# marqo-ai/marqo

Hardware: AMD Instinct MI355X
Metric: embeddings/sec (higher is better)
Workload: dtype bf16; 1 GPU; open_clip ViT-B/32 image tower, uint8 224x224 resident in HBM (tower-only), batch 256/GPU; global_batch=256, parallelism=dp1 (replicated weights, sharded items, RCCL all_gather of embeddings), weights=random-init (seed 0) ViT-B-32, last_block_rows=pooled

## Files before the change

marqo_amd/csrc/attn_proj.hip:

```cpp
#include "common.h"
#include "gemm_loop.h"

typedef short s16x4 __attribute__((ext_vector_type(4)));
typedef unsigned u32x2 __attribute__((ext_vector_type(2)));

extern mq_knob mq_xcd_band;
extern mq_knob mq_ln_prefetch;
int mq_device_ok();

namespace {

template <int OFF>
__device__ __forceinline__ s16x4 lds_read_tr16(unsigned addr) {
    s16x4 v;
    asm volatile("ds_read_b64_tr_b16 %0, %1 offset:%2" : "=v"(v) : "v"(addr), "n"(OFF));
    return v;
}
template <int OFF>
__device__ __forceinline__ bf16x8 gload16(const void* p) {
    i32x4 v;
    asm volatile("global_load_dwordx4 %0, %1, off offset:%2" : "=v"(v) : "v"(p), "n"(OFF));
    return __builtin_bit_cast(bf16x8, v);
}
struct ApPrefetch { const unsigned* a; const unsigned* b; unsigned na, nb; };
__device__ __forceinline__ void lds_write8(unsigned addr, u32x2 v) { asm volatile("ds_write_b64 %0, %1" ::"v"(addr), "v"(v) : "memory"); }

__device__ __forceinline__ float fold_sum(float v) {
    const auto r = __builtin_amdgcn_permlane16_swap(__float_as_uint(v), __float_as_uint(v), false, false);
    const float w = __uint_as_float(r[0]) + __uint_as_float(r[1]);
    const auto q = __builtin_amdgcn_permlane32_swap(__float_as_uint(w), __float_as_uint(w), false, false);
    return __uint_as_float(q[0]) + __uint_as_float(q[1]);
}
__device__ __forceinline__ float fold_max(float v) {
    const auto r = __builtin_amdgcn_permlane16_swap(__float_as_uint(v), __float_as_uint(v), false, false);
    const float w = fmaxf(__uint_as_float(r[0]), __uint_as_float(r[1]));
    const auto q = __builtin_amdgcn_permlane32_swap(__float_as_uint(w), __float_as_uint(w), false, false);
    return fmaxf(__uint_as_float(q[0]), __uint_as_float(q[1]));
}

constexpr int AP_TILE = 8192;
constexpr int AP_KV = 32768;
constexpr int AP_RING = 65536;

template <int W>
__global__ __launch_bounds__(512, 1) void attn_proj_kernel(const bf16_t* __restrict__ qkv, const bf16_t* __restrict__ Wo, const float* __restrict__ bias,
                                                            bf16_t* x, float2* __restrict__ rowstats, int len, float scale_log2e, float inv_w, float eps, int band, ApPrefetch pf, int dbg) {
    static_assert(W % 256 == 0 && (W / 64) % 2 == 0, "whole 256-column thirds, heads in pairs");
    constexpr int NHEAD = W / 64, NG = NHEAD / 2, NT3 = W / 256;
    constexpr int PANEL = NHEAD * AP_TILE;
    extern __shared__ __attribute__((aligned(16))) char smem[];
    const int tid = threadIdx.x, lane = tid & 63;
    const int wave = __builtin_amdgcn_readfirstlane(tid >> 6);
    const int l15 = lane & 15, g = lane >> 4;
    const unsigned img = xcd_banded_block(blockIdx.x, gridDim.x, band);
    const int64_t row0 = (int64_t)img * len;
    constexpr int ld = 3 * W;
    const bf16_t* qkv0 = qkv + row0 * ld;
    const unsigned lds0 = (unsigned)(uintptr_t)(__attribute__((address_space(3))) char*)smem;
    const unsigned ring = lds0 + PANEL;

    const int hl = wave >> 2, qblk = wave & 3;
    const bool active = qblk * 16 < len;
    auto stage = [&](int grp) {
        char* buf = smem + PANEL + (grp & 1) * AP_KV;
#pragma unroll
        for (int i = 0; i < 4; ++i) {
            const int p = wave * 4 + i;
            const int ph = p >> 4, is_v = (p >> 3) & 1, piece = p & 7;
            const int row = piece * 8 + (lane >> 3);
            const int key = row < len ? row : len - 1;
            const int lc = (lane & 7) ^ (row & 7);
            const bf16_t* src = qkv0 + (int64_t)key * ld + (is_v ? 2 * W : W) + (2 * grp + ph) * 64 + lc * 8;
            __builtin_amdgcn_global_load_lds((const __attribute__((address_space(1))) void*)src,
                                             (__attribute__((address_space(3))) void*)(buf + ph * 16384 + is_v * 8192 + piece * 1024), 16, 0, 0);
        }
    };
    const int qi = qblk * 16 + l15;
    const int64_t q_off = (int64_t)(qi < len ? qi : len - 1) * ld + hl * 64 + 8 * g;
    auto load_q = [&](int grp, bf16x8 (&q)[2]) {
        const bf16_t* qb = qkv0 + q_off + grp * 128;
        q[0] = gload16<0>(qb);
        q[1] = gload16<64>(qb);
    };
    const unsigned k_sw0 = (unsigned)(l15 * 128 + ((g ^ (l15 & 7)) << 4)), k_sw1 = (unsigned)(l15 * 128 + (((g + 4) ^ (l15 & 7)) << 4));
    const int vkey = 4 * g + (l15 >> 2), vcol = (l15 & 3) >> 1, vhalf = (l15 & 1) << 3;
    unsigned v_off[4];
#pragma unroll
    for (int dt = 0; dt < 4; ++dt) v_off[dt] = (unsigned)(8192 + vkey * 128 + ((((dt << 1) | vcol) ^ (vkey & 7)) << 4) + vhalf);
    unsigned o_off[4];
#pragma unroll
    for (int dt = 0; dt < 4; ++dt) o_off[dt] = (unsigned)(qi * 128 + (((dt * 2 + (g >> 1)) ^ (qi & 7)) << 4) + (g & 1) * 8);

    i32x4 res[4][NT3];
#pragma unroll
    for (int mt = 0; mt < 4; ++mt)
#pragma unroll
        for (int a = 0; a < NT3; ++a) res[mt][a] = i32x4{0, 0, 0, 0};
    unsigned pf_reg[2] = {0u, 0u};
    const unsigned pf_nt = gridDim.x * 512u, pf_t = blockIdx.x * 512u + (unsigned)tid;

    bf16x8 qn[2] = {bf16x8{0, 0, 0, 0, 0, 0, 0, 0}, bf16x8{0, 0, 0, 0, 0, 0, 0, 0}};
    if (!(dbg & 1)) {
    stage(0);
    load_q(0, qn);
    asm volatile("s_waitcnt vmcnt(0)" ::: "memory");
    landed(qn[0]); landed(qn[1]);
    static_for<NG>([&](auto grp_tag) {
        constexpr int grp = decltype(grp_tag)::value;
        __builtin_amdgcn_s_barrier();
        asm volatile("" ::: "memory");
        bf16x8 qf[2] = {qn[0], qn[1]};
        if constexpr (grp + 1 < NG) {
            stage(grp + 1);
            load_q(grp + 1, qn);
        }
        if constexpr (grp < 4) {
            const int m = grp * 16 + l15;
            const bf16_t* xr = x + (row0 + (m < len ? m : 0)) * W + wave * (W / 8) + (g & 1) * 16 + (g >> 1) * 8;
            static_for<NT3>([&](auto a_tag) {
                constexpr int a = decltype(a_tag)::value;
                res[grp][a] = __builtin_bit_cast(i32x4, gload16<a * 64>(xr));
            });
        }
        if constexpr (grp == 1 || grp == 3) {
            constexpr int j = grp >> 1;
// ... 89 lines not shown
    asm volatile("s_waitcnt lgkmcnt(0)" ::: "memory");
    __builtin_amdgcn_s_barrier();
    asm volatile("" ::: "memory");

    const unsigned slot0 = ring + (unsigned)wave * 8192u;
    const unsigned w_rd0 = (unsigned)(l15 * 128 + ((g ^ (l15 & 7)) << 4)), w_rd1 = (unsigned)(l15 * 128 + (((g + 4) ^ (l15 & 7)) << 4));
    const unsigned w_vo = (unsigned)((lane >> 3) * (W * 2) + (((lane & 7) ^ ((lane >> 3) & 7)) << 4));
    constexpr unsigned W_BYTES = (unsigned)W * W * 2;
    auto issue_unit = [&](int kt, int i, int slot, bool live) {
        const unsigned rec = live ? W_BYTES : 0u;
        const unsigned soff = (unsigned)((wave * (W / 8) + i * 16) * (W * 2) + kt * 128);
        const auto rs = __builtin_amdgcn_make_buffer_rsrc((void*)Wo, 0, rec, 0x00020000);
        dma16(rs, w_vo, soff, slot0 + (unsigned)slot * 2048u);
        dma16(rs, w_vo + 8u * (W * 2), soff, slot0 + (unsigned)slot * 2048u + 1024u);
    };
    f32x4 acc[NT3][4][2];
#pragma unroll
    for (int a = 0; a < NT3; ++a)
#pragma unroll
        for (int mt = 0; mt < 4; ++mt) { acc[a][mt][0] = f32x4{0.f, 0.f, 0.f, 0.f}; acc[a][mt][1] = f32x4{0.f, 0.f, 0.f, 0.f}; }
    constexpr int UPK = 2 * NT3;
    constexpr int UPI = 2 * UPK;
    static_assert(UPI % 4 == 0, "slot indices must be static inside an iteration");
    bf16x8 tf[4][2], wf[2][2];
    issue_unit(0, 0, 0, true);
    issue_unit(0, 1, 1, true);
    issue_unit(0, 2, 2, true);
    issue_unit(0, 3, 3, true);
    static_for<4>([&](auto mt_tag) {
        constexpr int mt = decltype(mt_tag)::value;
        tf[mt][0] = lds_read16<mt * 2048>(lds0 + w_rd0);
        tf[mt][1] = lds_read16<mt * 2048>(lds0 + w_rd1);
    });
    asm volatile("s_waitcnt vmcnt(6)" ::: "memory");
    wf[0][0] = lds_read16<0>(slot0 + w_rd0);
    wf[0][1] = lds_read16<0>(slot0 + w_rd1);
    for (int ktp = 0; ktp < ((dbg & 2) ? 0 : NHEAD / 2); ++ktp) {
        static_for<UPI>([&](auto ii_tag) {
            constexpr int ii = decltype(ii_tag)::value, i = ii % UPK, cur = ii & 1, slot = ii & 3;
            const int kt = 2 * ktp + ii / UPK;
            asm volatile("s_waitcnt lgkmcnt(0)" ::: "memory");
            landed(wf[cur][0]); landed(wf[cur][1]);
            if constexpr (i == 0) {
#pragma unroll
                for (int mt = 0; mt < 4; ++mt) { landed(tf[mt][0]); landed(tf[mt][1]); }
            }
            __builtin_amdgcn_sched_barrier(0);
            constexpr int a = i >> 1, j = i & 1;
#pragma unroll
            for (int mt = 0; mt < 4; ++mt) {
                acc[a][mt][j] = __builtin_amdgcn_mfma_f32_16x16x32_bf16(wf[cur][0], tf[mt][0], acc[a][mt][j], 0, 0, 0);
                acc[a][mt][j] = __builtin_amdgcn_mfma_f32_16x16x32_bf16(wf[cur][1], tf[mt][1], acc[a][mt][j], 0, 0, 0);
            }
            __builtin_amdgcn_sched_barrier(0);
            {
                constexpr int i4 = (ii + 4) % UPI;
                const int ktp4 = ktp + (ii + 4) / UPI;
                issue_unit(2 * ktp4 + i4 / UPK, i4 % UPK, slot, ktp4 < NHEAD / 2);
            }
            asm volatile("s_waitcnt vmcnt(6)" ::: "memory");
            {
                constexpr int nslot = (ii + 1) & 3;
                wf[cur ^ 1][0] = lds_read16<nslot * 2048>(slot0 + w_rd0);
                wf[cur ^ 1][1] = lds_read16<nslot * 2048>(slot0 + w_rd1);
            }
            if constexpr (i == UPK - 1) {
                __builtin_amdgcn_sched_barrier(0);
                const unsigned tb = lds0 + (unsigned)(kt + 1 < NHEAD ? kt + 1 : kt) * AP_TILE;
                static_for<4>([&](auto mt_tag) {
                    constexpr int mt = decltype(mt_tag)::value;
                    tf[mt][0] = lds_read16<mt * 2048>(tb + w_rd0);
                    tf[mt][1] = lds_read16<mt * 2048>(tb + w_rd1);
                });
            }
        });
    }
    asm volatile("s_waitcnt vmcnt(0)" ::: "memory");
    asm volatile("s_waitcnt lgkmcnt(0)" ::: "memory");
    landed(wf[0][0]); landed(wf[0][1]); landed(wf[1][0]); landed(wf[1][1]);
#pragma unroll
    for (int mt = 0; mt < 4; ++mt) { landed(tf[mt][0]); landed(tf[mt][1]); }

    if (dbg & 4) return;
    constexpr int WC = W / 8;
    f32x4 bias_v[NT3][2];
#pragma unroll
    for (int a = 0; a < NT3; ++a)
#pragma unroll
        for (int j = 0; j < 2; ++j) bias_v[a][j] = *(const f32x4*)(bias + wave * WC + a * 32 + j * 16 + 4 * g);
    char* mine = smem + PANEL + wave * 8192;
    const bool odd = (wave & 1) != 0;
    auto chain_add = [](f32x2_t& s1, f32x2_t& s2, unsigned px, unsigned py) {
        const f32x2_t e0 = {__uint_as_float(px << 16), __uint_as_float(px & 0xffff0000u)}, e1 = {__uint_as_float(py << 16), __uint_as_float(py & 0xffff0000u)};
        s1 += e0 + e1;
        s2 = __builtin_elementwise_fma(e0, e0, __builtin_elementwise_fma(e1, e1, s2));
    };
    unsigned held[4][4];
#pragma unroll
    for (int mt = 0; mt < 4; ++mt) {
        const int m = mt * 16 + l15;
        const bool m_ok = m < len;
        bf16_t* xr = x + (row0 + (m_ok ? m : 0)) * W + wave * WC;
        f32x2_t w1 = {0.f, 0.f}, w2 = {0.f, 0.f};
        f32x2_t h1 = {0.f, 0.f}, h2 = {0.f, 0.f};
#pragma unroll
        for (int a = 0; a < NT3; ++a) {
            uint2 pk[2];
            const auto q0 = __builtin_amdgcn_permlane16_swap((unsigned)res[mt][a][0], (unsigned)res[mt][a][2], false, false);
            const auto q1 = __builtin_amdgcn_permlane16_swap((unsigned)res[mt][a][1], (unsigned)res[mt][a][3], false, false);
#pragma unroll
            for (int j = 0; j < 2; ++j) {
                f32x4 v = acc[a][mt][j];
                v += bias_v[a][j];
                const unsigned rq[2] = {q0[j], q1[j]};
                v += f32x4{__uint_as_float(rq[0] << 16), __uint_as_float(rq[0] & 0xffff0000u), __uint_as_float(rq[1] << 16), __uint_as_float(rq[1] & 0xffff0000u)};
                pk[j].x = pack_bf16x2(v[0], v[1]);
                pk[j].y = pack_bf16x2(v[2], v[3]);
                const unsigned px = m_ok ? pk[j].x : 0u, py = m_ok ? pk[j].y : 0u;
                if constexpr (NT3 == 3) {
                    if (a == 1) chain_add(w1, w2, px, py);
                    else if (a == 0) {
                        if (odd) { held[mt][2 * j] = px; held[mt][2 * j + 1] = py; }
                        else chain_add(w1, w2, px, py);
                    } else {
                        if (odd) chain_add(w1, w2, px, py);
                        else chain_add(h1, h2, px, py);
                    }
                }
            }
            const auto r0 = __builtin_amdgcn_permlane16_swap(pk[0].x, pk[1].x, false, false);
            const auto r1 = __builtin_amdgcn_permlane16_swap(pk[0].y, pk[1].y, false, false);
            if (m_ok) *(uint4*)(xr + a * 32 + (g & 1) * 16 + (g >> 1) * 8) = make_uint4(r0[0], r1[0], r0[1], r1[1]);
        }
        if (rowstats) {
            const float st1 = fold_sum(w1[0] + w1[1]), st2 = fold_sum(w2[0] + w2[1]);
            if (g == 0) ((float2*)mine)[m] = make_float2(st1, st2);
            if (!odd) ((f32x4*)(mine + 1024))[mt * 64 + lane] = f32x4{h1[0], h1[1], h2[0], h2[1]};
        }
    }
    if (rowstats) {
        static_assert(NT3 == 3, "the slot hand-over is written for 96 columns per wave");
        __syncthreads();
        if (odd) {
            const f32x4* theirs = (const f32x4*)(smem + PANEL + (wave - 1) * 8192 + 1024);
#pragma unroll
            for (int mt = 0; mt < 4; ++mt) {
                const f32x4 st = theirs[mt * 64 + lane];
                f32x2_t h1 = {st[0], st[1]}, h2 = {st[2], st[3]};
                chain_add(h1, h2, held[mt][0], held[mt][1]);
                chain_add(h1, h2, held[mt][2], held[mt][3]);
                const float st1 = fold_sum(h1[0] + h1[1]), st2 = fold_sum(h2[0] + h2[1]);
                if (g == 0) ((float2*)(mine + 512))[mt * 16 + l15] = make_float2(st1, st2);
            }
        }
        __syncthreads();
        if (tid < len) {
            float s1 = 0.f, s2 = 0.f;
#pragma unroll
            for (int slot = 0; slot < W / 64; ++slot) {
                const int k = slot / 3, r = slot % 3;
                const char* src = smem + PANEL + (2 * k + (r ? 1 : 0)) * 8192 + (r == 1 ? 512 : 0);
                const float2 p = ((const float2*)src)[tid];
                s1 += p.x;
                s2 += p.y;
            }
            rowstats[row0 + tid] = mq_finalize_stats(s1, s2, inv_w, eps);
        }
    }
}

}

extern "C" int mq_attention_proj_ok(int64_t nseq, int32_t fixed_len, int32_t W, int32_t heads) {
    return nseq >= 1 && fixed_len >= 1 && fixed_len <= 64 && W == 768 && heads == 12 && nseq * fixed_len < (1LL << 31);
}

extern "C" int mq_attention_proj(const void* d_qkv, const void* d_w, const float* d_bias, void* d_x, float* d_rowstats, int64_t nseq, int32_t fixed_len, int32_t W,
                                 int32_t heads, float eps, const void* d_pf_a, size_t pf_a_bytes, const void* d_pf_b, size_t pf_b_bytes, void* stream) {
    MQ_CHECK_ARG(d_qkv && d_w && d_bias && d_x, "mq_attention_proj: null operand");
    MQ_CHECK_ARG(mq_attention_proj_ok(nseq, fixed_len, W, heads), "mq_attention_proj: takes 1..64-token sequences of a 768-wide tower with 12 heads (nseq=%ld len=%d W=%d heads=%d)",
                 (long)nseq, fixed_len, W, heads);
    MQ_CHECK_ARG((((uintptr_t)d_qkv | (uintptr_t)d_w | (uintptr_t)d_x | (uintptr_t)d_bias) & 15) == 0, "mq_attention_proj: operands must be 16-byte aligned");
    MQ_TRY(mq_device_ok());
    hipStream_t s = (hipStream_t)stream;
    constexpr int LDS = 12 * AP_TILE + AP_RING;
    static std::atomic<uint64_t> attr_done{0};
    auto kern = attn_proj_kernel<768>;
    if (hipError_t e = mq_ensure_dyn_lds((const void*)kern, LDS, attr_done); e != hipSuccess) {
        mq_set_error("mq_attention_proj: hipFuncSetAttribute: %s", hipGetErrorString(e));
        return MQ_ERR_HIP;
    }
    ApPrefetch pf{nullptr, nullptr, 0u, 0u};
    if (mq_ln_prefetch && nseq * fixed_len >= 1024) {
        auto lines = [](const void* p, size_t b) { return (p && ((uintptr_t)p & 3) == 0 && b < ((size_t)1 << 30)) ? (unsigned)(b / 128) : 0u; };
        pf.a = (const unsigned*)d_pf_a; pf.na = lines(d_pf_a, pf_a_bytes);
        pf.b = (const unsigned*)d_pf_b; pf.nb = lines(d_pf_b, pf_b_bytes);
    }
    static const bool dbg_on = getenv("MQ_AP_DEBUG") != nullptr;
    const char* dbg_s = dbg_on ? getenv("MQ_AP_DEBUG") : nullptr;
    const int dbg = dbg_s ? atoi(dbg_s) : 0;
    MqProfScope prof(2, s);
    const float scale_log2e = 1.44269504088896340736f / sqrtf(64.0f);
    hipLaunchKernelGGL(kern, dim3((unsigned)nseq), dim3(512), LDS, s, (const bf16_t*)d_qkv, (const bf16_t*)d_w, d_bias, (bf16_t*)d_x, (float2*)d_rowstats, (int)fixed_len,
                       scale_log2e, 1.0f / (float)W, eps, (mq_xcd_band && nseq >= 256) ? 1 : 0, pf, dbg);
    MQ_CHECK_LAUNCH("mq_attention_proj");
    return MQ_OK;
}
```

marqo_amd/csrc/gemm_bf16.hip:

```cpp
#include <map>
#include <mutex>
#include <string>
#include <type_traits>
#include "common.h"
#include "gemm_epilogue.h"
#include "gemm_loop.h"
#include "gemm_sched.h"

extern mq_knob mq_tower_row_select;
extern mq_knob mq_tower_ln_fold;
extern mq_knob mq_tower_subln_fold;
extern mq_knob mq_tower_attn_proj;
extern mq_knob mq_tower_panel_gemm;
extern mq_knob mq_attention_waves;
extern mq_knob mq_tower_residual_bf16;
extern mq_knob mq_gemm_small_max_rows;
bool mq_gemm_small_ok(int64_t M, int64_t N, int64_t K, bool ln);
bool mq_gemm_small_grouped_ok(int64_t M, int64_t N, int64_t K);
extern mq_knob mq_gemm_small_group_rows;
extern mq_knob mq_ln_prefetch;
int mq_gemm_small(const void* d_A, int64_t lda, const void* d_W, int64_t ldw, const float* d_bias, const void* d_residual, void* d_out,
                  int64_t ldc, int64_t M, int64_t N, int64_t K, int flags, hipStream_t s);
int mq_gemm_wd_launch(int flags, int mt, int ns, const void* A, int64_t lda, const void* W, int64_t ldw, const float* bias, const float* residual, void* out,
                      int64_t ldc, int M, int N, int K, const GemmGeom& g, int wide, const GemmLn& ln, hipStream_t s);

int mq_device_ok();

namespace {

struct GemmSk {
    float* partials;
    unsigned* flags;
    unsigned epoch;
    int tail_splits;
};

template <int FLAGS, int MT, int NH, int WM, int ORD>
__global__ __launch_bounds__(128 * WM, (NH == 1 && WM == 2) ? 2 : 1) void gemm_nt_kernel(
    const bf16_t* __restrict__ A, int64_t lda, const bf16_t* __restrict__ Wt, int64_t ldw,
    const float* __restrict__ bias, const float* residual, void* out, int64_t ldc,
    int M, int N, int K, int tiles_n, int num_tiles, int cgroup, int band_rows, int wide_store,
    unsigned a_bytes, unsigned w_bytes, GemmLn ln, GemmSk sk) {
    static_assert(!(NH == 2 && WM == 2), "the 4-wave 224 x 256 tile (one wave per SIMD) lost on every shape (profiles/r05a, r05b) and was removed in round 6");
    constexpr int BM = 16 * MT * WM, BN = 128 * NH;
    constexpr bool TAIL = WM == 4;
    constexpr int NTW = 4 * NH;
    constexpr int A_TILE_BYTES = BM * BK * 2, W_TILE_BYTES = BN * BK * 2;
    constexpr int STAGE_BYTES = A_TILE_BYTES + W_TILE_BYTES;
    constexpr int NPA = MT, NPW = 8 * NH / WM;
    constexpr int NLD = NPA + NPW;
    constexpr int NLR = MT + NTW;
    constexpr int NM = NTW * MT;
    constexpr bool LN_RES = (FLAGS & MQ_EPI_LN_APPLY) && (FLAGS & MQ_EPI_RESIDUAL);
    constexpr int ERG = !(FLAGS & MQ_EPI_RESIDUAL) ? MT : LN_RES ? ((NH == 2 || WM == 4) ? 1 : MT <= 4 ? MT : 2) : (NH == 2 || WM == 4) ? MT
                        : (FLAGS & MQ_EPI_OUT_F32) ? (MT <= 3 ? MT : (MT + 1) / 2) : (MT <= 5 ? MT : 3);
    extern __shared__ __attribute__((aligned(16))) char smem[];

    const GemmTileMap<BM, BN> tile_map(num_tiles, tiles_n, M, cgroup, band_rows);

    const int tid = threadIdx.x;
    const int lane = tid & 63;
    const int wave = __builtin_amdgcn_readfirstlane(tid >> 6);
    const int wm = wave >> 1, wn = wave & 1;
    const int l15 = lane & 15, g = lane >> 4;

    const int srow = lane >> 3;
    const unsigned chunk_off = (unsigned)(((lane & 7) ^ (srow & 7)) * 16);
    unsigned a_vo[NPA], w_vo[NPW];
    auto set_sources = [&](int m0, int n0) {
#pragma unroll
        for (int i = 0; i < MT; ++i) {
            int gm = m0 + wave * (8 * MT) + i * 8 + srow; gm = gm < M ? gm : M - 1;
            a_vo[i] = (unsigned)gm * (unsigned)lda * 2u + chunk_off;
        }
#pragma unroll
        for (int i = 0; i < NPW; ++i) {
            int gn = n0 + wave * (8 * NPW) + i * 8 + srow; gn = gn < N ? gn : N - 1;
            w_vo[i] = (unsigned)gn * (unsigned)ldw * 2u + chunk_off;
        }
    };
    const int nk = K / BK;
    int d_vbid = blockIdx.x, d_k = 0;
    unsigned a_rec = a_bytes, w_rec = w_bytes;
    bool tail_mode = false;
    int d_left = 0;
    const bool has_main = !TAIL || (int)blockIdx.x < num_tiles;
    if (has_main) {
        int m0, n0;
        tile_map.origin(d_vbid, m0, n0);
        set_sources(m0, n0);
    } else {
        a_rec = 0; w_rec = 0;
#pragma unroll
        for (int i = 0; i < NPA; ++i) a_vo[i] = 0;
#pragma unroll
        for (int i = 0; i < NPW; ++i) w_vo[i] = 0;
    }
    const unsigned lds0 = (unsigned)(uintptr_t)(__attribute__((address_space(3))) char*)smem;
    const unsigned dma_a0 = lds0 + (unsigned)wave * (8 * MT * 128), dma_w0 = lds0 + A_TILE_BYTES + (unsigned)wave * (8 * NPW * 128);
    auto issue_piece = [&](int i, unsigned bufoff) {
        const unsigned soff = (unsigned)d_k * (BK * 2);
        if (i < NPA) dma16(__builtin_amdgcn_make_buffer_rsrc((void*)A, 0, a_rec, 0x00020000), a_vo[i < NPA ? i : 0], soff, dma_a0 + bufoff + (unsigned)i * 1024u);
        else dma16(__builtin_amdgcn_make_buffer_rsrc((void*)Wt, 0, w_rec, 0x00020000), w_vo[i >= NPA ? i - NPA : 0], soff, dma_w0 + bufoff + (unsigned)(i - NPA) * 1024u);
// ... 493 lines not shown
    MqProfScope prof(0, s, 2.0 * (double)M * (double)N * (double)K);
    GemmLn ln{};
    ln.partials = (float2*)d_partials;
    ln.nslots = (int)((N + 63) / 64);
    ln.part_ld = M;
    return launch_gemm<MQ_EPI_BIAS | MQ_EPI_RESIDUAL | MQ_EPI_ROW_STATS>(d_A, lda, d_W, ldw, d_bias, (const float*)d_residual, d_out, ldc, (int)M, (int)N, (int)K, s, ln);
}

extern "C" int mq_gemm_bf16_lnrs(const void* d_A, int64_t lda, const void* d_W, int64_t ldw, const float* d_bias, const float* d_colsum, const float* d_rowstats,
                                 const void* d_residual, void* d_out, int64_t ldc, int64_t M, int64_t N, int64_t K, int flags, float* d_partials, void* stream) {
    MQ_CHECK_ARG(d_A && d_W && d_out && d_bias && d_colsum && d_rowstats && d_partials, "mq_gemm_bf16_lnrs: null operand");
    MQ_CHECK_ARG(flags == (MQ_EPI_BIAS | MQ_EPI_RESIDUAL) || flags == (MQ_EPI_BIAS | MQ_EPI_GLU), "mq_gemm_bf16_lnrs: flags must be MQ_EPI_BIAS | MQ_EPI_RESIDUAL or MQ_EPI_BIAS | MQ_EPI_GLU");
    MQ_CHECK_ARG(!(flags & MQ_EPI_RESIDUAL) || d_residual, "mq_gemm_bf16_lnrs: MQ_EPI_RESIDUAL without residual");
    MQ_TRY(check_shape("mq_gemm_bf16_lnrs", M, N, K, lda, ldw, ldc));
    MQ_CHECK_ARG(!(flags & MQ_EPI_GLU) || N % 32 == 0, "mq_gemm_bf16_lnrs: MQ_EPI_GLU needs N %% 32 == 0");
    hipStream_t s = (hipStream_t)stream;
    MqProfScope prof(0, s, 2.0 * (double)M * (double)N * (double)K);
    GemmLn ln{};
    ln.colsum = d_colsum;
    ln.rowstats = (const float2*)d_rowstats;
    ln.partials = (float2*)d_partials;
    ln.nslots = (int)((N + 63) / 64);
    ln.part_ld = M;
    if (flags & MQ_EPI_GLU)
        return launch_gemm<MQ_EPI_BIAS | MQ_EPI_GLU | MQ_EPI_LN_APPLY | MQ_EPI_ROW_STATS>(d_A, lda, d_W, ldw, d_bias, nullptr, d_out, ldc, (int)M, (int)N, (int)K, s, ln);
    return launch_gemm<MQ_EPI_BIAS | MQ_EPI_RESIDUAL | MQ_EPI_LN_APPLY | MQ_EPI_ROW_STATS>(d_A, lda, d_W, ldw, d_bias, (const float*)d_residual, d_out, ldc, (int)M, (int)N, (int)K, s, ln);
}

int mq_row_stats_finalize_pf(const float* d_partials, int32_t nslots, float* d_stats, int64_t rows, int32_t W, float eps, const void* pf_a, size_t bytes_a,
                             const void* pf_b, size_t bytes_b, hipStream_t s);
extern "C" int64_t mq_gemm_band_counters(int64_t M) { return M / 32 + 16; }
bool mq_gemm_rs_in_launch() { return g_tune.rs_fin && !g_tune.tail; }
extern "C" int mq_gemm_bf16_rsf(const void* d_A, int64_t lda, const void* d_W, int64_t ldw, const float* d_bias, const void* d_residual, void* d_out,
                                int64_t ldc, int64_t M, int64_t N, int64_t K, int flags, float* d_partials, float* d_stats, float eps,
                                uint32_t* d_band_ctr, const void* d_pf_a, size_t pf_a_bytes, const void* d_pf_b, size_t pf_b_bytes, void* stream) {
    MQ_CHECK_ARG(d_A && d_W && d_out && d_bias && d_residual && d_partials && d_stats, "mq_gemm_bf16_rsf: null operand");
    MQ_CHECK_ARG((flags | MQ_EPI_ROW_STATS) == (MQ_EPI_BIAS | MQ_EPI_RESIDUAL | MQ_EPI_ROW_STATS), "mq_gemm_bf16_rsf: flags must be MQ_EPI_BIAS | MQ_EPI_RESIDUAL");
    MQ_TRY(check_shape("mq_gemm_bf16_rsf", M, N, K, lda, ldw, ldc));
    hipStream_t s = (hipStream_t)stream;
    const int nslots = (int)((N + 63) / 64);
    const bool in_launch = d_band_ctr && g_tune.rs_fin && !g_tune.tail;
    {
        MqProfScope prof(0, s, 2.0 * (double)M * (double)N * (double)K);
        GemmLn ln{};
        ln.partials = (float2*)d_partials;
        ln.nslots = nslots;
        ln.part_ld = M;
        if (in_launch) {
            ln.band_ctr = d_band_ctr;
            ln.stats_out = (float2*)d_stats;
            ln.inv_w = 1.0f / (float)N;
            ln.eps = eps;
            ln.pf_a = (const unsigned*)d_pf_a;
            ln.pf_b = (const unsigned*)d_pf_b;
            ln.pf_na = d_pf_a ? (unsigned)(pf_a_bytes / 128) : 0u;
            ln.pf_nb = d_pf_b ? (unsigned)(pf_b_bytes / 128) : 0u;
        }
        MQ_TRY(launch_gemm<MQ_EPI_BIAS | MQ_EPI_RESIDUAL | MQ_EPI_ROW_STATS>(d_A, lda, d_W, ldw, d_bias, (const float*)d_residual, d_out, ldc, (int)M, (int)N, (int)K, s, ln));
    }
    if (in_launch) return MQ_OK;
    return mq_row_stats_finalize_pf(d_partials, nslots, d_stats, M, (int32_t)N, eps, d_pf_a, pf_a_bytes, d_pf_b, pf_b_bytes, s);
}

extern "C" int mq_tune(const char* key, int value) {
    MQ_CHECK_ARG(key, "mq_tune: null key");
    const std::string k(key);
    if (k == "gemm_mt") g_tune.mt = value;
    else if (k == "gemm_cgroup") g_tune.cgroup = value;
    else if (k == "gemm_nh") { g_tune.nh = value; g_tune.fp8_big = value == 4 ? 0 : value; }
    else if (k == "gemm_tail") g_tune.tail = value;
    else if (k == "gemm_wd") g_tune.wd = value;
    else if (k == "rs_finalize") g_tune.rs_fin = value;
    else if (k == "row_select") mq_tower_row_select = value;
    else if (k == "ln_fold") mq_tower_ln_fold = value;
    else if (k == "subln_fold") mq_tower_subln_fold = value;
    else if (k == "attn_proj") mq_tower_attn_proj = value;
    else if (k == "panel_gemm") mq_tower_panel_gemm = value;
    else if (k == "xcd_band") mq_xcd_band = value;
    else if (k == "attn_waves") mq_attention_waves = value;
    else if (k == "residual_bf16") mq_tower_residual_bf16 = value;
    else if (k == "small_m") mq_gemm_small_max_rows = value;
    else if (k == "small_m_grouped") mq_gemm_small_group_rows = value;
    else if (k == "ln_prefetch") mq_ln_prefetch = value;
    else if (k == "gemm_addr_limit_mb") mq_gemm_addr_limit = value > 0 ? ((uint64_t)value << 20) - 1 : 0xffffffffull;
    else { mq_set_error("mq_tune: unknown key %s", key); return MQ_ERR_INVALID; }
    return MQ_OK;
}
#endif
```

Before: 98150 embeddings/s.

## Interleave attention head-pairs with out-projection GEMM in fused attn_proj kernel

```diff
diff --git a/marqo_amd/csrc/attn_proj.hip b/marqo_amd/csrc/attn_proj.hip
--- a/marqo_amd/csrc/attn_proj.hip
+++ b/marqo_amd/csrc/attn_proj.hip
@@ -7,6 +7,7 @@
 extern mq_knob mq_xcd_band;
 extern mq_knob mq_ln_prefetch;
 int mq_device_ok();
+mq_knob mq_attn_proj_overlap{getenv("MQ_ATTN_PROJ_OVERLAP") ? atoi(getenv("MQ_ATTN_PROJ_OVERLAP")) : 1};
 
 namespace {
 
@@ -41,6 +42,97 @@
 constexpr int AP_TILE = 8192;
 constexpr int AP_KV = 32768;
 constexpr int AP_RING = 65536;
+
+template <int W>
+__device__ __forceinline__ void ap_epilogue(f32x4 (&acc)[W / 256][4][2], i32x4 (&res)[4][W / 256], const float* __restrict__ bias, bf16_t* x, float2* __restrict__ rowstats,
+                                            int64_t row0, int len, float inv_w, float eps, char* scratch, int tid, int lane, int wave, int l15, int g) {
+    constexpr int NT3 = W / 256;
+    constexpr int WC = W / 8;
+    f32x4 bias_v[NT3][2];
+#pragma unroll
+    for (int a = 0; a < NT3; ++a)
+#pragma unroll
+        for (int j = 0; j < 2; ++j) bias_v[a][j] = *(const f32x4*)(bias + wave * WC + a * 32 + j * 16 + 4 * g);
+    char* mine = scratch + wave * 8192;
+    const bool odd = (wave & 1) != 0;
+    auto chain_add = [](f32x2_t& s1, f32x2_t& s2, unsigned px, unsigned py) {
+        const f32x2_t e0 = {__uint_as_float(px << 16), __uint_as_float(px & 0xffff0000u)}, e1 = {__uint_as_float(py << 16), __uint_as_float(py & 0xffff0000u)};
+        s1 += e0 + e1;
+        s2 = __builtin_elementwise_fma(e0, e0, __builtin_elementwise_fma(e1, e1, s2));
+    };
+    unsigned held[4][4];
+#pragma unroll
+    for (int mt = 0; mt < 4; ++mt) {
+        const int m = mt * 16 + l15;
+        const bool m_ok = m < len;
+        bf16_t* xr = x + (row0 + (m_ok ? m : 0)) * W + wave * WC;
+        f32x2_t w1 = {0.f, 0.f}, w2 = {0.f, 0.f};
+        f32x2_t h1 = {0.f, 0.f}, h2 = {0.f, 0.f};
+#pragma unroll
+        for (int a = 0; a < NT3; ++a) {
+            uint2 pk[2];
+            const auto q0 = __builtin_amdgcn_permlane16_swap((unsigned)res[mt][a][0], (unsigned)res[mt][a][2], false, false);
+            const auto q1 = __builtin_amdgcn_permlane16_swap((unsigned)res[mt][a][1], (unsigned)res[mt][a][3], false, false);
+#pragma unroll
+            for (int j = 0; j < 2; ++j) {
+                f32x4 v = acc[a][mt][j];
+                v += bias_v[a][j];
+                const unsigned rq[2] = {q0[j], q1[j]};
+                v += f32x4{__uint_as_float(rq[0] << 16), __uint_as_float(rq[0] & 0xffff0000u), __uint_as_float(rq[1] << 16), __uint_as_float(rq[1] & 0xffff0000u)};
+                pk[j].x = pack_bf16x2(v[0], v[1]);
+                pk[j].y = pack_bf16x2(v[2], v[3]);
+                const unsigned px = m_ok ? pk[j].x : 0u, py = m_ok ? pk[j].y : 0u;
+                if constexpr (NT3 == 3) {
+                    if (a == 1) chain_add(w1, w2, px, py);
+                    else if (a == 0) {
+                        if (odd) { held[mt][2 * j] = px; held[mt][2 * j + 1] = py; }
+                        else chain_add(w1, w2, px, py);
+                    } else {
+                        if (odd) chain_add(w1, w2, px, py);
+                        else chain_add(h1, h2, px, py);
+                    }
+                }
+            }
+            const auto r0 = __builtin_amdgcn_permlane16_swap(pk[0].x, pk[1].x, false, false);
+            const auto r1 = __builtin_amdgcn_permlane16_swap(pk[0].y, pk[1].y, false, false);
+            if (m_ok) *(uint4*)(xr + a * 32 + (g & 1) * 16 + (g >> 1) * 8) = make_uint4(r0[0], r1[0], r0[1], r1[1]);
+        }
+        if (rowstats) {
+            const float st1 = fold_sum(w1[0] + w1[1]), st2 = fold_sum(w2[0] + w2[1]);
+            if (g == 0) ((float2*)mine)[m] = make_float2(st1, st2);
+            if (!odd) ((f32x4*)(mine + 1024))[mt * 64 + lane] = f32x4{h1[0], h1[1], h2[0], h2[1]};
+        }
+    }
+    if (rowstats) {
+        static_assert(NT3 == 3, "the slot hand-over is written for 96 columns per wave");
+        __syncthreads();
+        if (odd) {
+            const f32x4* theirs = (const f32x4*)(scratch + (wave - 1) * 8192 + 1024);
+#pragma unroll
+            for (int mt = 0; mt < 4; ++mt) {
+                const f32x4 st = theirs[mt * 64 + lane];
+                f32x2_t h1 = {st[0], st[1]}, h2 = {st[2], st[3]};
+                chain_add(h1, h2, held[mt][0], held[mt][1]);
+                chain_add(h1, h2, held[mt][2], held[mt][3]);
+                const float st1 = fold_sum(h1[0] + h1[1]), st2 = fold_sum(h2[0] + h2[1]);
+                if (g == 0) ((float2*)(mine + 512))[mt * 16 + l15] = make_float2(st1, st2);
+            }
+        }
+        __syncthreads();
+        if (tid < len) {
+            float s1 = 0.f, s2 = 0.f;
+#pragma unroll
+            for (int slot = 0; slot < W / 64; ++slot) {
+                const int k = slot / 3, r = slot % 3;
+                const char* src = scratch + (2 * k + (r ? 1 : 0)) * 8192 + (r == 1 ? 512 : 0);
+                const float2 p = ((const float2*)src)[tid];
+                s1 += p.x;
+                s2 += p.y;
+            }
+            rowstats[row0 + tid] = mq_finalize_stats(s1, s2, inv_w, eps);
+        }
+    }
+}
 
 template <int W>
 __global__ __launch_bounds__(512, 1) void attn_proj_kernel(const bf16_t* __restrict__ qkv, const bf16_t* __restrict__ Wo, const float* __restrict__ bias,
@@ -296,91 +388,293 @@
     for (int mt = 0; mt < 4; ++mt) { landed(tf[mt][0]); landed(tf[mt][1]); }
 
     if (dbg & 4) return;
-    constexpr int WC = W / 8;
-    f32x4 bias_v[NT3][2];
+    ap_epilogue<W>(acc, res, bias, x, rowstats, row0, len, inv_w, eps, smem + PANEL, tid, lane, wave, l15, g);
+}
+
+template <int W, int DBG>
+__global__ __launch_bounds__(512, 1) void attn_proj_overlap_kernel(const bf16_t* __restrict__ qkv, const bf16_t* __restrict__ Wo, const float* __restrict__ bias,
+                                                                    bf16_t* x, float2* __restrict__ rowstats, int len, float scale_log2e, float inv_w, float eps, int band, ApPrefetch pf) {
+    static_assert(W % 256 == 0 && (W / 64) % 2 == 0, "whole 256-column thirds, heads in pairs");
+    constexpr int NHEAD = W / 64, NG = NHEAD / 2, NT3 = W / 256;
+    constexpr int OBUF = 4 * AP_TILE;
+    constexpr int KVOFF = OBUF, RINGOFF = OBUF + 2 * AP_KV;
+    extern __shared__ __attribute__((aligned(16))) char smem[];
+    const int tid = threadIdx.x, lane = tid & 63;
+    const int wave = __builtin_amdgcn_readfirstlane(tid >> 6);
+    const int l15 = lane & 15, g = lane >> 4;
+    const unsigned img = xcd_banded_block(blockIdx.x, gridDim.x, band);
+    const int64_t row0 = (int64_t)img * len;
+    constexpr int ld = 3 * W;
+    const bf16_t* qkv0 = qkv + row0 * ld;
+    const unsigned lds0 = (unsigned)(uintptr_t)(__attribute__((address_space(3))) char*)smem;
+
+    const int hl = wave >> 2, qblk = wave & 3;
+    const bool active = qblk * 16 < len;
+    auto stage = [&](int grp, int half) {
+        char* buf = smem + KVOFF + (grp & 1) * AP_KV;
+#pragma unroll
+        for (int i = 2 * half; i < 2 * half + 2; ++i) {
+            const int p = wave * 4 + i;
+            const int ph = p >> 4, is_v = (p >> 3) & 1, piece = p & 7;
+            const int row = piece * 8 + (lane >> 3);
+            const int key = row < len ? row : len - 1;
+            const int lc = (lane & 7) ^ (row & 7);
+            const unsigned off = (unsigned)(key * ld + (is_v ? 2 * W : W) + ph * 64 + lc * 8) * 2u;
+            const char* src = (const char*)qkv0 + off + grp * 256;
+            __builtin_amdgcn_global_load_lds((const __attribute__((address_space(1))) void*)src,
+                                             (__attribute__((address_space(3))) void*)(buf + ph * 16384 + is_v * 8192 + piece * 1024), 16, 0, 0);
+        }
+    };
+    const int qi = qblk * 16 + l15;
+    const unsigned q_off = (unsigned)((qi < len ? qi : len - 1) * ld + hl * 64 + 8 * g) * 2u;
+    auto load_q = [&](int grp, bf16x8 (&q)[2]) {
+        const char* qb = (const char*)qkv0 + q_off + grp * 256;
+        q[0] = gload16<0>(qb);
+        q[1] = gload16<64>(qb);
+    };
+    const unsigned k_sw0 = (unsigned)(l15 * 128 + ((g ^ (l15 & 7)) << 4));
+    const int vkey = 4 * g + (l15 >> 2), vcol = (l15 & 3) >> 1, vhalf = (l15 & 1) << 3;
+    const unsigned v_off0 = (unsigned)(8192 + vkey * 128 + ((vcol ^ (vkey & 7)) << 4) + vhalf);
+    const unsigned o_off0 = (unsigned)(qi * 128 + (((g >> 1) ^ (qi & 7)) << 4) + (g & 1) * 8);
+
+    constexpr int RES0 = NG - 2;
+    i32x4 res[4][NT3];
+#pragma unroll
+    for (int mt = 0; mt < 4; ++mt)
+#pragma unroll
+        for (int a = 0; a < NT3; ++a) res[mt][a] = i32x4{0, 0, 0, 0};
+    unsigned pf_reg[2] = {0u, 0u};
+    const unsigned pf_nt = gridDim.x * 512u, pf_t = blockIdx.x * 512u + (unsigned)tid;
+
+    const unsigned slot0 = lds0 + RINGOFF + (unsigned)wave * 8192u;
+    const unsigned w_vo = (unsigned)((lane >> 3) * (W * 2) + (((lane & 7) ^ ((lane >> 3) & 7)) << 4));
+    constexpr unsigned W_BYTES = (unsigned)W * W * 2;
+    auto issue_unit = [&](int kt, int i, int slot, bool live) {
+        const unsigned rec = live ? W_BYTES : 0u;
+        const unsigned soff = (unsigned)((wave * (W / 8) + i * 16) * (W * 2) + kt * 128);
+        const auto rs = __builtin_amdgcn_make_buffer_rsrc((void*)Wo, 0, rec, 0x00020000);
+        dma16(rs, w_vo, soff, slot0 + (unsigned)slot * 2048u);
+        dma16(rs, w_vo + 8u * (W * 2), soff, slot0 + (unsigned)slot * 2048u + 1024u);
+    };
+    f32x4 acc[NT3][4][2];
 #pragma unroll
     for (int a = 0; a < NT3; ++a)
 #pragma unroll
-        for (int j = 0; j < 2; ++j) bias_v[a][j] = *(const f32x4*)(bias + wave * WC + a * 32 + j * 16 + 4 * g);
-    char* mine = smem + PANEL + wave * 8192;
-    const bool odd = (wave & 1) != 0;
-    auto chain_add = [](f32x2_t& s1, f32x2_t& s2, unsigned px, unsigned py) {
-        const f32x2_t e0 = {__uint_as_float(px << 16), __uint_as_float(px & 0xffff0000u)}, e1 = {__uint_as_float(py << 16), __uint_as_float(py & 0xffff0000u)};
-        s1 += e0 + e1;
-        s2 = __builtin_elementwise_fma(e0, e0, __builtin_elementwise_fma(e1, e1, s2));
-    };
-    unsigned held[4][4];
-#pragma unroll
-    for (int mt = 0; mt < 4; ++mt) {
-        const int m = mt * 16 + l15;
-        const bool m_ok = m < len;
-        bf16_t* xr = x + (row0 + (m_ok ? m : 0)) * W + wave * WC;
-        f32x2_t w1 = {0.f, 0.f}, w2 = {0.f, 0.f};
-        f32x2_t h1 = {0.f, 0.f}, h2 = {0.f, 0.f};
-#pragma unroll
-        for (int a = 0; a < NT3; ++a) {
-            uint2 pk[2];
-            const auto q0 = __builtin_amdgcn_permlane16_swap((unsigned)res[mt][a][0], (unsigned)res[mt][a][2], false, false);
-            const auto q1 = __builtin_amdgcn_permlane16_swap((unsigned)res[mt][a][1], (unsigned)res[mt][a][3], false, false);
-#pragma unroll
-            for (int j = 0; j < 2; ++j) {
-                f32x4 v = acc[a][mt][j];
-                v += bias_v[a][j];
-                const unsigned rq[2] = {q0[j], q1[j]};
-                v += f32x4{__uint_as_float(rq[0] << 16), __uint_as_float(rq[0] & 0xffff0000u), __uint_as_float(rq[1] << 16), __uint_as_float(rq[1] & 0xffff0000u)};
-                pk[j].x = pack_bf16x2(v[0], v[1]);
-                pk[j].y = pack_bf16x2(v[2], v[3]);
-                const unsigned px = m_ok ? pk[j].x : 0u, py = m_ok ? pk[j].y : 0u;
-                if constexpr (NT3 == 3) {
-                    if (a == 1) chain_add(w1, w2, px, py);
-                    else if (a == 0) {
-                        if (odd) { held[mt][2 * j] = px; held[mt][2 * j + 1] = py; }
-                        else chain_add(w1, w2, px, py);
-                    } else {
-                        if (odd) chain_add(w1, w2, px, py);
-                        else chain_add(h1, h2, px, py);
+        for (int mt = 0; mt < 4; ++mt) { acc[a][mt][0] = f32x4{0.f, 0.f, 0.f, 0.f}; acc[a][mt][1] = f32x4{0.f, 0.f, 0.f, 0.f}; }
+    constexpr int UPK = 2 * NT3;
+    constexpr int UPR = 2 * UPK;
+    static_assert(UPR % 4 == 0 && UPR > 4, "slot indices must be static inside a round");
+    constexpr bool LOADS = !(DBG & 1), ATTN = !(DBG & 1) && !(DBG & 8), UNITS = !(DBG & 2);
+
+    bf16x8 qn[2] = {bf16x8{0, 0, 0, 0, 0, 0, 0, 0}, bf16x8{0, 0, 0, 0, 0, 0, 0, 0}};
+    bf16x8 tf[4][2], wf[2][2];
+    if constexpr (LOADS) {
+        stage(0, 0);
+        stage(0, 1);
+        load_q(0, qn);
+    }
+    if constexpr (UNITS) {
+        issue_unit(0, 0, 0, true);
+        issue_unit(0, 1, 1, true);
+        issue_unit(0, 2, 2, true);
+        issue_unit(0, 3, 3, true);
+    }
+    asm volatile("s_waitcnt vmcnt(0)" ::: "memory");
+    landed(qn[0]); landed(qn[1]);
+    if constexpr (UNITS) {
+        wf[0][0] = lds_read16<0>(slot0 + k_sw0);
+        wf[0][1] = lds_read16<0>(slot0 + (k_sw0 ^ 64u));
+    }
+    static_for<NG + 1>([&](auto r_tag) {
+        constexpr int r = decltype(r_tag)::value;
+        if constexpr (r == 1) asm volatile("s_waitcnt lgkmcnt(0)" ::: "memory");
+        __builtin_amdgcn_s_barrier();
+        asm volatile("" ::: "memory");
+        constexpr int n_a = !LOADS ? 0 : (r + 1 < NG ? 2 : 0) + (r == NG ? 2 * NT3 : r >= RES0 ? NT3 : 0) + ((r == 1 || r == 3) ? 1 : 0);
+        constexpr int n_b = (LOADS && r + 1 < NG) ? 4 : 0;
+        auto issue_b = [&]() {
+            if constexpr (n_b != 0) {
+                stage(r + 1, 1);
+                load_q(r + 1, qn);
+            }
+        };
+        if constexpr (LOADS) {
+            if constexpr (r + 1 < NG) stage(r + 1, 0);
+            if constexpr (r >= RES0) {
+                static_for<(r == NG ? 2 : 1)>([&](auto t_tag) {
+                    constexpr int mt = r - RES0 + decltype(t_tag)::value;
+                    const int m = mt * 16 + l15;
+                    const char* xr = (const char*)(x + row0 * W) + (unsigned)((m < len ? m : 0) * W + wave * (W / 8) + (g & 1) * 16 + (g >> 1) * 8) * 2u;
+                    static_for<NT3>([&](auto a_tag) {
+                        constexpr int a = decltype(a_tag)::value;
+                        res[mt][a] = __builtin_bit_cast(i32x4, gload16<a * 64>(xr));
+                    });
+                });
+            }
+            if constexpr (r == 1 || r == 3) {
+                constexpr int j = r >> 1;
+                const unsigned c = pf_t + j * pf_nt;
+                const unsigned* src = c < pf.na ? pf.a + (size_t)c * 32 : (c - pf.na < pf.nb ? pf.b + (size_t)(c - pf.na) * 32 : (const unsigned*)qkv0);
+                asm volatile("global_load_dword %0, %1, off" : "=v"(pf_reg[j]) : "v"(src));
+            }
+        }
+        auto b_landed = [&]() { landed(qn[0]); landed(qn[1]); };
+        auto a_landed = [&]() {
+            if constexpr (LOADS && r >= RES0) {
+#pragma unroll
+                for (int a = 0; a < NT3; ++a) landed(res[r - RES0][a]);
+                if constexpr (r == NG) {
+#pragma unroll
+                    for (int a = 0; a < NT3; ++a) landed(res[r - RES0 + 1][a]);
+                }
+            }
+            if constexpr (LOADS && (r == 1 || r == 3)) landed(pf_reg[r >> 1]);
+        };
+        if constexpr (ATTN && r < NG) {
+            if (active) {
+                const unsigned kvb = lds0 + KVOFF + (unsigned)(r & 1) * AP_KV + (unsigned)hl * 16384u;
+                f32x4 sc[4];
+                static_for<2>([&](auto h_tag) {
+                    constexpr int h = decltype(h_tag)::value;
+                    bf16x8 kf[2][2];
+                    static_for<2>([&](auto t_tag) {
+                        constexpr int t = decltype(t_tag)::value;
+                        kf[t][0] = lds_read16<(2 * h + t) * 2048>(kvb + k_sw0);
+                        kf[t][1] = lds_read16<(2 * h + t) * 2048>(kvb + (k_sw0 ^ 64u));
+                    });
+                    asm volatile("s_waitcnt lgkmcnt(0)" ::: "memory");
+#pragma unroll
+                    for (int t = 0; t < 2; ++t) {
+                        landed(kf[t][0]); landed(kf[t][1]);
+                        sc[2 * h + t] = f32x4{0.f, 0.f, 0.f, 0.f};
+#pragma unroll
+                        for (int kk = 0; kk < 2; ++kk) sc[2 * h + t] = __builtin_amdgcn_mfma_f32_16x16x32_bf16(kf[t][kk], qn[kk], sc[2 * h + t], 0, 0, 0);
                     }
-                }
-            }
-            const auto r0 = __builtin_amdgcn_permlane16_swap(pk[0].x, pk[1].x, false, false);
-            const auto r1 = __builtin_amdgcn_permlane16_swap(pk[0].y, pk[1].y, false, false);
-            if (m_ok) *(uint4*)(xr + a * 32 + (g & 1) * 16 + (g >> 1) * 8) = make_uint4(r0[0], r1[0], r0[1], r1[1]);
-        }
-        if (rowstats) {
-            const float st1 = fold_sum(w1[0] + w1[1]), st2 = fold_sum(w2[0] + w2[1]);
-            if (g == 0) ((float2*)mine)[m] = make_float2(st1, st2);
-            if (!odd) ((f32x4*)(mine + 1024))[mt * 64 + lane] = f32x4{h1[0], h1[1], h2[0], h2[1]};
-        }
-    }
-    if (rowstats) {
-        static_assert(NT3 == 3, "the slot hand-over is written for 96 columns per wave");
-        __syncthreads();
-        if (odd) {
-            const f32x4* theirs = (const f32x4*)(smem + PANEL + (wave - 1) * 8192 + 1024);
-#pragma unroll
-            for (int mt = 0; mt < 4; ++mt) {
-                const f32x4 st = theirs[mt * 64 + lane];
-                f32x2_t h1 = {st[0], st[1]}, h2 = {st[2], st[3]};
-                chain_add(h1, h2, held[mt][0], held[mt][1]);
-                chain_add(h1, h2, held[mt][2], held[mt][3]);
-                const float st1 = fold_sum(h1[0] + h1[1]), st2 = fold_sum(h2[0] + h2[1]);
-                if (g == 0) ((float2*)(mine + 512))[mt * 16 + l15] = make_float2(st1, st2);
-            }
-        }
-        __syncthreads();
-        if (tid < len) {
-            float s1 = 0.f, s2 = 0.f;
-#pragma unroll
-            for (int slot = 0; slot < W / 64; ++slot) {
-                const int k = slot / 3, r = slot % 3;
-                const char* src = smem + PANEL + (2 * k + (r ? 1 : 0)) * 8192 + (r == 1 ? 512 : 0);
-                const float2 p = ((const float2*)src)[tid];
-                s1 += p.x;
-                s2 += p.y;
-            }
-            rowstats[row0 + tid] = mq_finalize_stats(s1, s2, inv_w, eps);
-        }
-    }
+                });
+                s16x4 vt[2][4];
+                auto read_v = [&](auto u_tag) {
+                    constexpr int u = decltype(u_tag)::value;
+                    static_for<4>([&](auto dt_tag) {
+                        constexpr int dt = decltype(dt_tag)::value;
+                        vt[0][dt] = lds_read_tr16<u * 4096>(kvb + (v_off0 ^ (unsigned)(dt << 5)));
+                        vt[1][dt] = lds_read_tr16<u * 4096 + 2048>(kvb + (v_off0 ^ (unsigned)(dt << 5)));
+                    });
+                };
+                read_v(std::integral_constant<int, 0>{});
+                if (len < 64) {
+#pragma unroll
+                    for (int t = 0; t < 4; ++t)
+#pragma unroll
+                        for (int q = 0; q < 4; ++q) sc[t][q] = (t * 16 + g * 4 + q < len) ? sc[t][q] : -INFINITY;
+                }
+                float mx = fmaxf(fmaxf(fmaxf(sc[0][0], sc[0][1]), fmaxf(sc[0][2], sc[0][3])), fmaxf(fmaxf(sc[1][0], sc[1][1]), fmaxf(sc[1][2], sc[1][3])));
+                mx = fmaxf(mx, fmaxf(fmaxf(fmaxf(sc[2][0], sc[2][1]), fmaxf(sc[2][2], sc[2][3])), fmaxf(fmaxf(sc[3][0], sc[3][1]), fmaxf(sc[3][2], sc[3][3]))));
+                mx = fold_max(mx);
+                const float neg_mc = -mx * scale_log2e;
+                float psum = 0.f;
+#pragma unroll
+                for (int t = 0; t < 4; ++t)
+#pragma unroll
+                    for (int q = 0; q < 4; ++q) {
+                        sc[t][q] = __builtin_amdgcn_exp2f(fmaf(sc[t][q], scale_log2e, neg_mc));
+                        psum += sc[t][q];
+                    }
+                f32x4 o[4];
+#pragma unroll
+                for (int dt = 0; dt < 4; ++dt) o[dt] = f32x4{0.f, 0.f, 0.f, 0.f};
+                static_for<2>([&](auto u_tag) {
+                    constexpr int u = decltype(u_tag)::value;
+                    asm volatile("s_waitcnt lgkmcnt(0)" ::: "memory");
+#pragma unroll
+                    for (int t = 0; t < 2; ++t)
+#pragma unroll
+                        for (int dt = 0; dt < 4; ++dt) landed(vt[t][dt]);
+                    union { uint32_t w[4]; bf16x8 v; } pb;
+                    pb.w[0] = pack_bf16x2(sc[2 * u][0], sc[2 * u][1]);
+                    pb.w[1] = pack_bf16x2(sc[2 * u][2], sc[2 * u][3]);
+                    pb.w[2] = pack_bf16x2(sc[2 * u + 1][0], sc[2 * u + 1][1]);
+                    pb.w[3] = pack_bf16x2(sc[2 * u + 1][2], sc[2 * u + 1][3]);
+#pragma unroll
+                    for (int dt = 0; dt < 4; ++dt) {
+                        union { s16x4 t[2]; bf16x8 v; } vf;
+                        vf.t[0] = vt[0][dt];
+                        vf.t[1] = vt[1][dt];
+                        o[dt] = __builtin_amdgcn_mfma_f32_16x16x32_bf16(vf.v, pb.v, o[dt], 0, 0, 0);
+                    }
+                    if constexpr (u == 0) {
+                        __builtin_amdgcn_sched_barrier(0);
+                        read_v(std::integral_constant<int, 1>{});
+                    }
+                });
+                const float inv = 1.0f / fold_sum(psum);
+                const unsigned ot = lds0 + (unsigned)(2 * (r & 1) + hl) * AP_TILE;
+#pragma unroll
+                for (int dt = 0; dt < 4; ++dt) {
+                    u32x2 p;
+                    p[0] = pack_bf16x2(o[dt][0] * inv, o[dt][1] * inv);
+                    p[1] = pack_bf16x2(o[dt][2] * inv, o[dt][3] * inv);
+                    lds_write8(ot + (o_off0 ^ (unsigned)(dt << 5)), p);
+                }
+            }
+        }
+        if constexpr (UNITS && r >= 1) {
+            constexpr unsigned ob = (unsigned)(2 * ((r - 1) & 1)) * AP_TILE;
+            static_for<4>([&](auto mt_tag) {
+                constexpr int mt = decltype(mt_tag)::value;
+                tf[mt][0] = lds_read16<mt * 2048>(lds0 + ob + k_sw0);
+                tf[mt][1] = lds_read16<mt * 2048>(lds0 + ob + (k_sw0 ^ 64u));
+            });
+            static_for<UPR>([&](auto ii_tag) {
+                constexpr int ii = decltype(ii_tag)::value, i = ii % UPK, cur = ii & 1, slot = ii & 3;
+                if constexpr (ii == UPK) issue_b();
+                asm volatile("s_waitcnt lgkmcnt(0)" ::: "memory");
+                landed(wf[cur][0]); landed(wf[cur][1]);
+                if constexpr (i == 0) {
+#pragma unroll
+                    for (int mt = 0; mt < 4; ++mt) { landed(tf[mt][0]); landed(tf[mt][1]); }
+                }
+                __builtin_amdgcn_sched_barrier(0);
+                constexpr int a = i >> 1, j = i & 1;
+#pragma unroll
+                for (int mt = 0; mt < 4; ++mt) {
+                    acc[a][mt][j] = __builtin_amdgcn_mfma_f32_16x16x32_bf16(wf[cur][0], tf[mt][0], acc[a][mt][j], 0, 0, 0);
+                    acc[a][mt][j] = __builtin_amdgcn_mfma_f32_16x16x32_bf16(wf[cur][1], tf[mt][1], acc[a][mt][j], 0, 0, 0);
+                }
+                __builtin_amdgcn_sched_barrier(0);
+                {
+                    constexpr int i4 = (ii + 4) % UPR, kt4 = 2 * (r - 1 + (ii + 4) / UPR) + i4 / UPK;
+                    issue_unit(kt4, i4 % UPK, slot, kt4 < NHEAD);
+                }
+                static_assert(6 + n_a < 32 && 6 + n_b < 32, "far inside the 6-bit counter");
+                asm volatile("s_waitcnt vmcnt(%0)" ::"n"(ii < 3 ? 6 + n_a : (ii >= UPK && ii < UPK + 3) ? 6 + n_b : 6) : "memory");
+                if constexpr (ii == 3) a_landed();
+                if constexpr (ii == UPK + 3) b_landed();
+                if constexpr (ii + 1 < UPR || r < NG) {
+                    constexpr int nslot = (ii + 1) & 3;
+                    wf[cur ^ 1][0] = lds_read16<nslot * 2048>(slot0 + k_sw0);
+                    wf[cur ^ 1][1] = lds_read16<nslot * 2048>(slot0 + (k_sw0 ^ 64u));
+                }
+                if constexpr (i == UPK - 1 && ii < UPR - 1) {
+                    __builtin_amdgcn_sched_barrier(0);
+                    static_for<4>([&](auto mt_tag) {
+                        constexpr int mt = decltype(mt_tag)::value;
+                        tf[mt][0] = lds_read16<AP_TILE + mt * 2048>(lds0 + ob + k_sw0);
+                        tf[mt][1] = lds_read16<AP_TILE + mt * 2048>(lds0 + ob + (k_sw0 ^ 64u));
+                    });
+                }
+            });
+        } else {
+            issue_b();
+            asm volatile("s_waitcnt vmcnt(0)" ::: "memory");
+            a_landed(); b_landed();
+        }
+    });
+    asm volatile("s_waitcnt vmcnt(0)" ::: "memory");
+    asm volatile("s_waitcnt lgkmcnt(0)" ::: "memory");
+    __builtin_amdgcn_sched_barrier(0);
+
+    if constexpr (DBG & 4) return;
+    ap_epilogue<W>(acc, res, bias, x, rowstats, row0, len, inv_w, eps, smem + RINGOFF, tid, lane, wave, l15, g);
 }
 
 }
@@ -398,12 +692,6 @@
     MQ_TRY(mq_device_ok());
     hipStream_t s = (hipStream_t)stream;
     constexpr int LDS = 12 * AP_TILE + AP_RING;
-    static std::atomic<uint64_t> attr_done{0};
-    auto kern = attn_proj_kernel<768>;
-    if (hipError_t e = mq_ensure_dyn_lds((const void*)kern, LDS, attr_done); e != hipSuccess) {
-        mq_set_error("mq_attention_proj: hipFuncSetAttribute: %s", hipGetErrorString(e));
-        return MQ_ERR_HIP;
-    }
     ApPrefetch pf{nullptr, nullptr, 0u, 0u};
     if (mq_ln_prefetch && nseq * fixed_len >= 1024) {
         auto lines = [](const void* p, size_t b) { return (p && ((uintptr_t)p & 3) == 0 && b < ((size_t)1 << 30)) ? (unsigned)(b / 128) : 0u; };
@@ -413,10 +701,41 @@
     static const bool dbg_on = getenv("MQ_AP_DEBUG") != nullptr;
     const char* dbg_s = dbg_on ? getenv("MQ_AP_DEBUG") : nullptr;
     const int dbg = dbg_s ? atoi(dbg_s) : 0;
-    MqProfScope prof(2, s);
     const float scale_log2e = 1.44269504088896340736f / sqrtf(64.0f);
-    hipLaunchKernelGGL(kern, dim3((unsigned)nseq), dim3(512), LDS, s, (const bf16_t*)d_qkv, (const bf16_t*)d_w, d_bias, (bf16_t*)d_x, (float2*)d_rowstats, (int)fixed_len,
-                       scale_log2e, 1.0f / (float)W, eps, (mq_xcd_band && nseq >= 256) ? 1 : 0, pf, dbg);
+    const int band = (mq_xcd_band && nseq >= 256) ? 1 : 0;
+    if (mq_attn_proj_overlap) {
+        using kern_t = void (*)(const bf16_t*, const bf16_t*, const float*, bf16_t*, float2*, int, float, float, float, int, ApPrefetch);
+        static std::atomic<uint64_t> attr_done[8];
+        int slot = 0;
+        kern_t kern = attn_proj_overlap_kernel<768, 0>;
+        switch (dbg) {
+            case 0: break;
+            case 1: kern = attn_proj_overlap_kernel<768, 1>; slot = 1; break;
+            case 2: kern = attn_proj_overlap_kernel<768, 2>; slot = 2; break;
+            case 3: kern = attn_proj_overlap_kernel<768, 3>; slot = 3; break;
+            case 4: kern = attn_proj_overlap_kernel<768, 4>; slot = 4; break;
+            case 7: kern = attn_proj_overlap_kernel<768, 7>; slot = 5; break;
+            case 8: kern = attn_proj_overlap_kernel<768, 8>; slot = 6; break;
+            default: mq_set_error("mq_attention_proj: MQ_AP_DEBUG=%d has no interleaved build (0, 1, 2, 3, 4, 7, 8)", dbg); return MQ_ERR_INVALID;
+        }
+        if (hipError_t e = mq_ensure_dyn_lds((const void*)kern, LDS, attr_done[slot]); e != hipSuccess) {
+            mq_set_error("mq_attention_proj: hipFuncSetAttribute: %s", hipGetErrorString(e));
+            return MQ_ERR_HIP;
+        }
+        MqProfScope prof(2, s);
+        hipLaunchKernelGGL(kern, dim3((unsigned)nseq), dim3(512), LDS, s, (const bf16_t*)d_qkv, (const bf16_t*)d_w, d_bias, (bf16_t*)d_x, (float2*)d_rowstats, (int)fixed_len,
+                           scale_log2e, 1.0f / (float)W, eps, band, pf);
+    } else {
+        static std::atomic<uint64_t> attr_done{0};
+        auto kern = attn_proj_kernel<768>;
+        if (hipError_t e = mq_ensure_dyn_lds((const void*)kern, LDS, attr_done); e != hipSuccess) {
+            mq_set_error("mq_attention_proj: hipFuncSetAttribute: %s", hipGetErrorString(e));
+            return MQ_ERR_HIP;
+        }
+        MqProfScope prof(2, s);
+        hipLaunchKernelGGL(kern, dim3((unsigned)nseq), dim3(512), LDS, s, (const bf16_t*)d_qkv, (const bf16_t*)d_w, d_bias, (bf16_t*)d_x, (float2*)d_rowstats, (int)fixed_len,
+                           scale_log2e, 1.0f / (float)W, eps, band, pf, dbg);
+    }
     MQ_CHECK_LAUNCH("mq_attention_proj");
     return MQ_OK;
 }
diff --git a/marqo_amd/csrc/gemm_bf16.hip b/marqo_amd/csrc/gemm_bf16.hip
--- a/marqo_amd/csrc/gemm_bf16.hip
+++ b/marqo_amd/csrc/gemm_bf16.hip
@@ -19,6 +19,7 @@
 bool mq_gemm_small_grouped_ok(int64_t M, int64_t N, int64_t K);
 extern mq_knob mq_gemm_small_group_rows;
 extern mq_knob mq_ln_prefetch;
+extern mq_knob mq_attn_proj_overlap;
 int mq_gemm_small(const void* d_A, int64_t lda, const void* d_W, int64_t ldw, const float* d_bias, const void* d_residual, void* d_out,
                   int64_t ldc, int64_t M, int64_t N, int64_t K, int flags, hipStream_t s);
 int mq_gemm_wd_launch(int flags, int mt, int ns, const void* A, int64_t lda, const void* W, int64_t ldw, const float* bias, const float* residual, void* out,
@@ -678,6 +679,7 @@
     else if (k == "small_m") mq_gemm_small_max_rows = value;
     else if (k == "small_m_grouped") mq_gemm_small_group_rows = value;
     else if (k == "ln_prefetch") mq_ln_prefetch = value;
+    else if (k == "attn_proj_overlap") mq_attn_proj_overlap = value;
     else if (k == "gemm_addr_limit_mb") mq_gemm_addr_limit = value > 0 ? ((uint64_t)value << 20) - 1 : 0xffffffffull;
     else { mq_set_error("mq_tune: unknown key %s", key); return MQ_ERR_INVALID; }
     return MQ_OK;
```

After: 99100 embeddings/s, median of 6. Within noise of the previous version (+1.0%).
